# AolinFeng/PMP-VVC-TIP2023

Hardware: AMD Instinct MI355X
Metric: CTUs/sec (luma QT+MTT inference+post-proc) (higher is better)
Workload: dtype f16x3

## Files before the change

### pmp_vvc_tip2023_amd/csrc/conv_f16x3.hip

```cpp
#include <cstdio>
#include <type_traits>

#include "pmp_kernels.h"
#include "split3.h"

namespace pmp {

template <int KH, int KW, int NTHR = 256>
struct StagePlanH {
    unsigned off[GeoH<KH, KW, 16, NTHR>::NLD];
    unsigned valid;
};

template <int KH, int KW, int NTHR = 256>
__device__ __forceinline__ void h2_plan(StagePlanH<KH, KW, NTHR> &p, size_t plane_stride, int H, int W, int ty, int tx)
{
    typedef GeoH<KH, KW, 16, NTHR> G;
    constexpr int PY = KH / 2, PX = KW / 2;
    p.valid = 0;
#pragma unroll
    for (int k = 0; k < G::NLD; ++k) {
        const int i = min((int)threadIdx.x + k * NTHR, G::PIECES - 1);
        const int sp = i / G::PLANE, j = i - sp * G::PLANE, pix = j >> 1, half = j & 1;
        const int row = pix / G::TW, col = pix - row * G::TW;
        const int gy = ty * 16 + row - PY, gx = tx * 16 + col - PX;
        const bool in = gy >= 0 && gy < H && gx >= 0 && gx < W && (int)threadIdx.x + k * NTHR < G::PIECES;
        if (in) p.valid |= 1u << k;
        const int cy = min(max(gy, 0), H - 1), cx = min(max(gx, 0), W - 1);
        p.off[k] = (unsigned)(sp * plane_stride + ((size_t)cy * W + cx) * 16 + half * 8);
    }
}

template <int KH, int KW, int NTHR = 256>
__device__ __forceinline__ void h2_stage_load(const StagePlanH<KH, KW, NTHR> &p, const unsigned short *__restrict__ grp,
                                              u32x4 (&r)[GeoH<KH, KW, 16, NTHR>::NLD], int k0 = 0, int k1 = 1 << 20)
{
#pragma unroll
    for (int k = 0; k < GeoH<KH, KW, 16, NTHR>::NLD; ++k) {
        if (k < k0 || k >= k1) continue;
        r[k] = *reinterpret_cast<const u32x4 *>(grp + p.off[k]);
    }
}

template <int KH, int KW, int NTHR = 256>
__device__ __forceinline__ void h2_stage_store(const StagePlanH<KH, KW, NTHR> &p, u32x4 *lds, const u32x4 (&r)[GeoH<KH, KW, 16, NTHR>::NLD],
                                               int k0 = 0, int k1 = 1 << 20)
{
    typedef GeoH<KH, KW, 16, NTHR> G;
#pragma unroll
    for (int k = 0; k < G::NLD; ++k) {
        if (k < k0 || k >= k1) continue;
        const int i = min((int)threadIdx.x + k * NTHR, G::PIECES);
        const u32x4 z = {0u, 0u, 0u, 0u};
        lds[i] = ((p.valid >> k) & 1u) ? r[k] : z;
    }
}

template <int KH, int KW, int NT, bool LEAN = false>
__device__ __forceinline__ void h2_accumulate(const unsigned short *__restrict__ x, size_t plane_stride,
                                              const unsigned short *__restrict__ wpk, int C, int H, int W, int n, int ty,
                                              int tx, u32x4 *lds, f32x4 (&acc)[WaveTile<NT>::RW][WaveTile<NT>::CW])
{
    constexpr int NTHR = 256;
    typedef GeoH<KH, KW, 16, NTHR> G;
    typedef WaveTile<NT> WT;
    constexpr int RW = WT::RW, CW = WT::CW;
    const int lane = threadIdx.x & 63, wave = threadIdx.x >> 6, xl = lane & 15, g = lane >> 4;
    const int rh = wave % WT::RSPLIT, ch = wave / WT::RSPLIT;
    const int CB = C >> 4;
    const size_t grp_sz = (size_t)H * W * 16;
    const unsigned short *grp0 = x + (size_t)n * CB * grp_sz;
    constexpr bool W0DB = NT == 4;
    constexpr bool W2 = W0DB && G::TAPS == 9 && !LEAN;
    u32x4 r[G::NLD];
    StagePlanH<KH, KW, NTHR> plan;
    const bool paired = (CB & 1) == 0 && (G::TAPS & 1);
    const f16x8 *wl = reinterpret_cast<const f16x8 *>(wpk) + lane + ch * CW * 64;
    const int last = paired ? (CB / 2) * G::TAPS - 1 : CB * G::NKS - 1;
    f16x8 w0[CW], w1[CW];
    f16x8 w0n[CW];
    f16x8 w1n[CW], w0nn[CW];
    h2_plan<KH, KW, NTHR>(plan, plane_stride, H, W, ty, tx);
#pragma unroll
    for (int nt = 0; nt < CW; ++nt) {
        if (W0DB) w0n[nt] = wl[(0 * NT + nt) * 64]; else w0[nt] = wl[(0 * NT + nt) * 64];
        w1[nt] = wl[(1 * NT + nt) * 64];
        if (W2) {
            const f16x8 *w2 = wl + (size_t)min(1, last) * (2 * NT * 64);
            w0nn[nt] = w2[(0 * NT + nt) * 64]; w1n[nt] = w2[(1 * NT + nt) * 64];
        }
    }
    __syncthreads();
    h2_stage_load<KH, KW, NTHR>(plan, grp0, r);
    h2_stage_store<KH, KW, NTHR>(plan, lds, r);
    __syncthreads();
    const int pb = ((rh * RW * G::TW + xl) * 2 + (g & 1)) * 16;
    int stream = 0;
    int tapsel = g >> 1;
    constexpr int O_LAST = (((G::TAPS - 1) / KW) * G::TW + (G::TAPS - 1) % KW) * 32;
    f16x8 x0[RW], x1[RW];

    auto group = [&](auto mode_tag, auto tail_tag, int cb) {
        constexpr int MODE = decltype(mode_tag)::value;
        constexpr int TAIL = decltype(tail_tag)::value;
        constexpr bool LAST = TAIL == 2;
        constexpr int NK = MODE == 0 ? G::NKS : (MODE == 1 ? (G::TAPS - 1) / 2 : (G::TAPS - 1) / 2 + 1);
        constexpr int PER = (G::NLD + (NK > 0 ? NK : 1) - 1) / (NK > 0 ? NK : 1);
        constexpr int LAG = G::TAPS > 9 ? 3 : 2;
        constexpr bool FETCH = TAIL < 2;
        u32x4 (&rl)[G::NLD] = r;
        u32x4 (&rs)[G::NLD] = r;
        constexpr bool more = !LAST;
        const unsigned short *nxt_grp = grp0 + (size_t)min(cb + 1, CB - 1) * grp_sz;
        const int bcur = cb & 1, bprev = (cb + 1) & 1;
        const char *buf = reinterpret_cast<const char *>(lds + bcur * G::BUF);
        auto xaddr = [&](int ks) -> const char * {
            const int j = MODE == 2 ? ks - 1 : ks;
            int tA = 2 * j, tB = 2 * j + 1;
            if (MODE == 0 && tB >= G::TAPS) tB = tA;
            const int oA = ((tA / KW) * G::TW + tA % KW) * 32, oB = ((tB / KW) * G::TW + tB % KW) * 32;
            return buf + (tapsel ? oB : oA) + pb;
        };
        if constexpr (LEAN) {
            constexpr int RS = 2, SUB = RW / RS;
            const char *part = reinterpret_cast<const char *>(lds + bprev * G::BUF);
            if (NK == 0 && FETCH) h2_stage_load<KH, KW, NTHR>(plan, nxt_grp, rl);
#pragma unroll
            for (int ks = 0; ks < NK; ++ks) {
                asm volatile("" : "+v"(tapsel));
                const char *px = (MODE == 2 && ks == 0) ? (g < 2 ? part : buf) + O_LAST + pb : xaddr(ks);
                ++stream;
                const f16x8 *wf = wl + (size_t)min(stream, last) * (2 * NT * 64);
                f16x8 xa[RS], xb[RS];
                auto rd_a = [&](int h) __attribute__((always_inline)) {
#pragma unroll
                    for (int m = 0; m < RS; ++m) xa[m] = *reinterpret_cast<const f16x8 *>(px + (h * RS + m) * G::TW * 32);
                };
                auto rd_b = [&](int h) __attribute__((always_inline)) {
#pragma unroll
                    for (int m = 0; m < RS; ++m) xb[m] = *reinterpret_cast<const f16x8 *>(px + G::PLANE * 16 + (h * RS + m) * G::TW * 32);
                };
#pragma unroll
                for (int h = 0; h < SUB; ++h) {
                    rd_a(h); rd_b(h);
                    __builtin_amdgcn_sched_barrier(0);
#pragma unroll
                    for (int m = 0; m < RS; ++m)
#pragma unroll
                        for (int nt = 0; nt < CW; ++nt)
                            acc[h * RS + m][nt] = __builtin_amdgcn_mfma_f32_16x16x32_f16(w1[nt], xa[m], acc[h * RS + m][nt], 0, 0, 0);
                    __builtin_amdgcn_sched_barrier(0);
                    if (h == 0) {
#pragma unroll
                        for (int nt = 0; nt < CW; ++nt) w0[nt] = w0n[nt];
#pragma unroll
                        for (int nt = 0; nt < CW; ++nt) { w1n[nt] = wf[(1 * NT + nt) * 64]; w0n[nt] = wf[(0 * NT + nt) * 64]; }
                        if (FETCH) h2_stage_load<KH, KW, NTHR>(plan, nxt_grp, rl, ks * PER, (ks + 1) * PER);
                        if (more && ks >= LAG)
                            h2_stage_store<KH, KW, NTHR>(plan, lds + ((cb + 1) & 1) * G::BUF, rs, (ks - LAG) * PER, (ks - LAG + 1) * PER);
                    } else if (h == SUB - 1) {
#pragma unroll
                        for (int nt = 0; nt < CW; ++nt) w1[nt] = w1n[nt];
                    }
                    __builtin_amdgcn_sched_barrier(0);
#pragma unroll
                    for (int m = 0; m < RS; ++m)
#pragma unroll
                        for (int nt = 0; nt < CW; ++nt)
                            acc[h * RS + m][nt] = __builtin_amdgcn_mfma_f32_16x16x32_f16(w0[nt], xa[m], acc[h * RS + m][nt], 0, 0, 0);
                    __builtin_amdgcn_sched_barrier(0);
#pragma unroll
                    for (int m = 0; m < RS; ++m)
#pragma unroll
                        for (int nt = 0; nt < CW; ++nt)
                            acc[h * RS + m][nt] = __builtin_amdgcn_mfma_f32_16x16x32_f16(w0[nt], xb[m], acc[h * RS + m][nt], 0, 0, 0);
                    __builtin_amdgcn_sched_barrier(0);
                }
                if (MODE == 2 && ks == 0) h2_lds_barrier();
            }
        } else {
            if (NK == 0) {
                if (FETCH) h2_stage_load<KH, KW, NTHR>(plan, nxt_grp, rl);
            } else if (MODE == 2) {
                if (g >= 2) {
                    const char *pl = buf + O_LAST + pb;
#pragma unroll
                    for (int m = 0; m < RW; ++m) {
                        x0[m] = *reinterpret_cast<const f16x8 *>(pl + m * G::TW * 32);
                        x1[m] = *reinterpret_cast<const f16x8 *>(pl + G::PLANE * 16 + m * G::TW * 32);
                    }
                }
            } else {
                const char *p0x = xaddr(0);
#pragma unroll
                for (int m = 0; m < RW; ++m) x0[m] = *reinterpret_cast<const f16x8 *>(p0x + m * G::TW * 32);
            }
#pragma unroll
            for (int ks = 0; ks < NK; ++ks) {
                asm volatile("" : "+v"(tapsel));
                const char *px = (MODE == 2 && ks == 0) ? buf : xaddr(ks);
                ++stream;
                if (!(MODE == 2 && ks == 0)) {
#pragma unroll
                    for (int m = 0; m < RW; ++m) x1[m] = *reinterpret_cast<const f16x8 *>(px + G::PLANE * 16 + m * G::TW * 32);
                }
                const f16x8 *wf = wl + (size_t)min(stream, last) * (2 * NT * 64);
                __builtin_amdgcn_sched_barrier(0);
#pragma unroll
                for (int m = 0; m < RW; ++m)
#pragma unroll
                    for (int nt = 0; nt < CW; ++nt) acc[m][nt] = __builtin_amdgcn_mfma_f32_16x16x32_f16(w1[nt], x0[m], acc[m][nt], 0, 0, 0);
                __builtin_amdgcn_sched_barrier(0);
                if (W2) {
                    const f16x8 *wf2 = wl + (size_t)min(stream + 1, last) * (2 * NT * 64);
#pragma unroll
                    for (int nt = 0; nt < CW; ++nt) { w1[nt] = w1n[nt]; w0[nt] = w0n[nt]; w0n[nt] = w0nn[nt]; }
#pragma unroll
                    for (int nt = 0; nt < CW; ++nt) w1n[nt] = wf2[(1 * NT + nt) * 64];
#pragma unroll
                    for (int nt = 0; nt < CW; ++nt) w0nn[nt] = wf2[(0 * NT + nt) * 64];
                } else {
#pragma unroll
                    for (int nt = 0; nt < CW; ++nt) w1[nt] = wf[(1 * NT + nt) * 64];
                    if (W0DB) {
#pragma unroll
                        for (int nt = 0; nt < CW; ++nt) w0[nt] = w0n[nt];
#pragma unroll
                        for (int nt = 0; nt < CW; ++nt) w0n[nt] = wf[(0 * NT + nt) * 64];
                    }
                }
                if (FETCH) h2_stage_load<KH, KW, NTHR>(plan, nxt_grp, rl, ks * PER, (ks + 1) * PER);
                if (more && ks >= LAG)
                    h2_stage_store<KH, KW, NTHR>(plan, lds + ((cb + 1) & 1) * G::BUF, rs, (ks - LAG) * PER, (ks - LAG + 1) * PER);
                __builtin_amdgcn_sched_barrier(0);
#pragma unroll
                for (int m = 0; m < RW; ++m)
#pragma unroll
                    for (int nt = 0; nt < CW; ++nt) acc[m][nt] = __builtin_amdgcn_mfma_f32_16x16x32_f16(w0[nt], x0[m], acc[m][nt], 0, 0, 0);
                __builtin_amdgcn_sched_barrier(0);
                if (ks + 1 < NK) {
                    const char *pn = xaddr(ks + 1);
#pragma unroll
                    for (int m = 0; m < RW; ++m) x0[m] = *reinterpret_cast<const f16x8 *>(pn + m * G::TW * 32);
                }
                __builtin_amdgcn_sched_barrier(0);
#pragma unroll
                for (int m = 0; m < RW; ++m)
#pragma unroll
                    for (int nt = 0; nt < CW; ++nt) acc[m][nt] = __builtin_amdgcn_mfma_f32_16x16x32_f16(w0[nt], x1[m], acc[m][nt], 0, 0, 0);
                __builtin_amdgcn_sched_barrier(0);
                if (!W0DB) {
#pragma unroll
                    for (int nt = 0; nt < CW; ++nt) w0[nt] = wf[(0 * NT + nt) * 64];
                }
                __builtin_amdgcn_sched_barrier(0);
            }
            if (MODE == 1 && g < 2) {
                const char *pl = buf + O_LAST + pb;
#pragma unroll
                for (int m = 0; m < RW; ++m) {
                    x0[m] = *reinterpret_cast<const f16x8 *>(pl + m * G::TW * 32);
                    x1[m] = *reinterpret_cast<const f16x8 *>(pl + G::PLANE * 16 + m * G::TW * 32);
                }
            }
        }
        if (more) h2_stage_store<KH, KW, NTHR>(plan, lds + ((cb + 1) & 1) * G::BUF, rs, NK > LAG ? (NK - LAG) * PER : 0);
        __syncthreads();
    };

    typedef std::integral_constant<int, 0> M0;
    typedef std::integral_constant<int, 1> M1;
    typedef std::integral_constant<int, 2> M2;
    typedef std::integral_constant<int, 0> T0;
    typedef std::integral_constant<int, 1> T1;
    typedef std::integral_constant<int, 2> T2;
    if (paired) {
        for (int cb = 0; cb + 2 < CB; cb += 2) {
            group(M1{}, T0{}, cb);
            group(M2{}, T0{}, cb + 1);
        }
        group(M1{}, T1{}, CB - 2);
        group(M2{}, T2{}, CB - 1);
    } else {
        for (int cb = 0; cb + 1 < CB; ++cb) group(M0{}, T0{}, cb);
        group(M0{}, T2{}, CB - 1);
    }
}

template <int NT>
__device__ __forceinline__ void h2_epilogue(const ConvX6Args &a, f32x4 (&acc)[WaveTile<NT>::RW][WaveTile<NT>::CW], int n, int ty, int tx);

template <int NT>
__device__ __forceinline__ void h2_shortcut32(const ConvX6Args &a, int n, int ty, int tx, u32x4 *lds,
                                              f32x4 (&acc)[WaveTile<NT>::RW][WaveTile<NT>::CW])
{
    typedef WaveTile<NT> WT;
    constexpr int RW = WT::RW, CW = WT::CW;
    const int tid = threadIdx.x, lane = tid & 63, wave = tid >> 6, xl = lane & 15, g = lane >> 4;
    const int rh = wave % WT::RSPLIT, ch = wave / WT::RSPLIT;
    const int W = a.W;
    const size_t grp_sz = (size_t)a.H * W * 16;
    const unsigned short *base = a.x_sc + (size_t)n * 2 * grp_sz + ((size_t)(ty * 16) * W + tx * 16) * 16;
    __syncthreads();
    u32x4 r[8];
#pragma unroll
    for (int k = 0; k < 8; ++k) {
        const int i = tid + k * 256, grp = i >> 10, plane = (i >> 9) & 1, j = i & 511, px = j >> 1, half = j & 1;
        r[k] = *reinterpret_cast<const u32x4 *>(base + plane * a.sc_stride + grp * grp_sz + ((size_t)(px >> 4) * W + (px & 15)) * 16 + half * 8);
    }
    const f16x8 *wl = reinterpret_cast<const f16x8 *>(a.w_sc) + lane + ch * CW * 64;
    f16x8 w0[CW], w1[CW];
#pragma unroll
    for (int nt = 0; nt < CW; ++nt) { w0[nt] = wl[(0 * NT + nt) * 64]; w1[nt] = wl[(1 * NT + nt) * 64]; }
#pragma unroll
    for (int k = 0; k < 8; ++k) lds[tid + k * 256] = r[k];
    __syncthreads();
    const char *px = reinterpret_cast<const char *>(lds) + (g >> 1) * 16384 + ((rh * RW * 16 + xl) * 2 + (g & 1)) * 16;
#pragma unroll
    for (int h = 0; h < RW / 2; ++h) {
        f16x8 xa[2], xb[2];
#pragma unroll
        for (int m = 0; m < 2; ++m) {
            xa[m] = *reinterpret_cast<const f16x8 *>(px + (h * 2 + m) * 16 * 32);
            xb[m] = *reinterpret_cast<const f16x8 *>(px + 8192 + (h * 2 + m) * 16 * 32);
        }
#pragma unroll
        for (int m = 0; m < 2; ++m)
#pragma unroll
            for (int nt = 0; nt < CW; ++nt) acc[h * 2 + m][nt] = __builtin_amdgcn_mfma_f32_16x16x32_f16(w1[nt], xa[m], acc[h * 2 + m][nt], 0, 0, 0);
#pragma unroll
        for (int m = 0; m < 2; ++m)
#pragma unroll
            for (int nt = 0; nt < CW; ++nt) acc[h * 2 + m][nt] = __builtin_amdgcn_mfma_f32_16x16x32_f16(w0[nt], xa[m], acc[h * 2 + m][nt], 0, 0, 0);
#pragma unroll
        for (int m = 0; m < 2; ++m)
#pragma unroll
            for (int nt = 0; nt < CW; ++nt) acc[h * 2 + m][nt] = __builtin_amdgcn_mfma_f32_16x16x32_f16(w0[nt], xb[m], acc[h * 2 + m][nt], 0, 0, 0);
    }
}

template <int KH, int KW, int NT, int SC, bool LEAN = false>
__global__ __launch_bounds__(256, NT == 4 && !LEAN ? 2 : 3) void conv_h2_kernel(ConvX6Args a)
{
    typedef GeoH<KH, KW> G;
    __shared__ u32x4 lds[2 * G::BUF];
    const int tiles_x = a.W >> 4, tiles = tiles_x * (a.H >> 4);
    int bid = blockIdx.x;
    if ((gridDim.x & 7) == 0) bid = (bid & 7) * (gridDim.x >> 3) + (bid >> 3);
    const int n = bid / tiles, t = bid - n * tiles, ty = t / tiles_x, tx = t - ty * tiles_x;
    typedef WaveTile<NT> WT;
    constexpr int RW = WT::RW, CW = WT::CW;

    f32x4 acc[RW][CW];
#pragma unroll
    for (int m = 0; m < RW; ++m)
#pragma unroll
        for (int nt = 0; nt < CW; ++nt) acc[m][nt] = (f32x4){0.f, 0.f, 0.f, 0.f};

    h2_accumulate<KH, KW, NT, LEAN>(a.x, a.x_stride, a.w, a.Cin, a.H, a.W, n, ty, tx, lds, acc);
    if (SC == 2) h2_shortcut32<NT>(a, n, ty, tx, lds, acc);
    else if (SC) h2_accumulate<1, 1, NT, LEAN>(a.x_sc, a.sc_stride, a.w_sc, a.Csc, a.H, a.W, n, ty, tx, lds, acc);
    h2_epilogue<NT>(a, acc, n, ty, tx);
}

template <int NT>
__device__ __forceinline__ void h2_epilogue(const ConvX6Args &a, f32x4 (&acc)[WaveTile<NT>::RW][WaveTile<NT>::CW], int n, int ty, int tx)
{
    typedef WaveTile<NT> WT;
    constexpr int RW = WT::RW, CW = WT::CW;
    int tid = threadIdx.x;
    asm volatile("" : "+v"(tid));
    const int lane = tid & 63, wave = tid >> 6, xl = lane & 15, g = lane >> 4;
    const int rh = wave % WT::RSPLIT, ch = wave / WT::RSPLIT;
    const int H = a.H, W = a.W;
    const size_t grp = (size_t)H * W * 16;

    const float inv_scale = a.out_scale;
    const unsigned off0 = (unsigned)(((size_t)n * NT + ch * CW) * grp + ((size_t)(ty * 16 + rh * RW) * W + tx * 16 + xl) * 16 + g * 4);
    const unsigned row_el = (unsigned)W * 16;
    const unsigned off0w = off0 - (unsigned)(g * 4) + (unsigned)(8 * (g >> 1)) + (unsigned)(g & 1) * row_el;
    u32x4 ra[RW / 2][CW], rbv[RW / 2][CW];
    auto res_load = [&](int nt, int slot) __attribute__((always_inline)) {
#pragma unroll
        for (int m = 0; m < RW; m += 2) {
            const unsigned off = off0w + (unsigned)m * row_el + (unsigned)nt * (unsigned)grp;
            ra[m >> 1][slot] = __builtin_nontemporal_load(reinterpret_cast<const u32x4 *>(a.res + off));
            rbv[m >> 1][slot] = __builtin_nontemporal_load(reinterpret_cast<const u32x4 *>(a.res + off + a.res_stride));
        }
    };
    auto res_add = [&](int nt, int slot) __attribute__((always_inline)) {
#pragma unroll
        for (int m = 0; m < RW; m += 2) {
            u32x4 p = ra[m >> 1][slot], q = rbv[m >> 1][slot];
            rows16_swap(p);
            rows16_swap(q);
            acc[m][nt] = acc[m][nt] * inv_scale + h2_sum4_lo(p, q);
            acc[m + 1][nt] = acc[m + 1][nt] * inv_scale + h2_sum4_hi(p, q);
        }
    };
    if (a.res) {
#pragma unroll
        for (int nt = 0; nt < CW; ++nt) res_load(nt, nt);
#pragma unroll
        for (int nt = 0; nt < CW; ++nt) res_add(nt, nt);
    } else {
#pragma unroll
        for (int nt = 0; nt < CW; ++nt)
#pragma unroll
            for (int m = 0; m < RW; ++m) acc[m][nt] = acc[m][nt] * inv_scale;
    }
    float amax = 0.f;
#pragma unroll
    for (int nt = 0; nt < CW; ++nt) {
#pragma unroll
        for (int m = 0; m < RW; ++m) {
            const unsigned off = off0 + (unsigned)m * row_el + (unsigned)nt * (unsigned)grp;
            f32x4 v = acc[m][nt];
            if (a.relu) { v.x = fmaxf(v.x, 0.f); v.y = fmaxf(v.y, 0.f); v.z = fmaxf(v.z, 0.f); v.w = fmaxf(v.w, 0.f); }
            if (a.gate) v *= load_split2_4(a.gate + off, a.gate_stride);
            amax = sat_amax4(amax, v);
            acc[m][nt] = v;
        }
        if (!a.pool) {
            if (a.out_f32) {
#pragma unroll
                for (int m = 0; m < RW; ++m)
                    *reinterpret_cast<f32x4 *>(a.out_f32 + off0 + (unsigned)m * row_el + (unsigned)nt * (unsigned)grp) = acc[m][nt];
            } else {
#pragma unroll
                for (int m = 0; m < RW; m += 2) {
                    const unsigned off = off0w + (unsigned)m * row_el + (unsigned)nt * (unsigned)grp;
                    u32x4 p, q;
                    split2_rows(acc[m][nt], acc[m + 1][nt], p, q);
                    rows16_swap(p);
                    rows16_swap(q);
                    __builtin_nontemporal_store(p, reinterpret_cast<u32x4 *>(a.out + off));
                    __builtin_nontemporal_store(q, reinterpret_cast<u32x4 *>(a.out + off + a.out_stride));
                }
            }
        } else {
            const int Ho = H >> 1, Wo = W >> 1;
#pragma unroll
            for (int m = 0; m < RW; m += 2) {
                f32x4 v = acc[m][nt], u = acc[m + 1][nt];
                v.x = fmaxf(v.x, u.x); v.y = fmaxf(v.y, u.y); v.z = fmaxf(v.z, u.z); v.w = fmaxf(v.w, u.w);
                f32x4 o;
                o.x = __shfl_xor(v.x, 1); o.y = __shfl_xor(v.y, 1); o.z = __shfl_xor(v.z, 1); o.w = __shfl_xor(v.w, 1);
                v.x = fmaxf(v.x, o.x); v.y = fmaxf(v.y, o.y); v.z = fmaxf(v.z, o.z); v.w = fmaxf(v.w, o.w);
                if ((xl & 1) == 0) {
                    const int yo = ty * 8 + rh * (RW / 2) + (m >> 1), xo = tx * 8 + (xl >> 1);
                    const size_t off = (((size_t)n * NT + ch * CW + nt) * Ho + yo) * Wo * 16 + (size_t)xo * 16 + g * 4;
                    if (a.out_f32) *reinterpret_cast<f32x4 *>(a.out_f32 + off) = v;
                    else store_split2_4(a.out + off, a.out_stride, v);
                }
            }
        }
    }
    if (!a.out_f32) sat_report(a.sat, amax);
}

#define PMP_H2_LAUNCH(NT)                                                                                       \
    if (a.x_sc) hipLaunchKernelGGL((conv_h2_kernel<KH, KW, NT, 1>), dim3(grid), dim3(256), 0, s, a);           \
    else hipLaunchKernelGGL((conv_h2_kernel<KH, KW, NT, 0>), dim3(grid), dim3(256), 0, s, a)

template <int KH, int KW>
static hipError_t launch_h2(hipStream_t s, const ConvX6Args &a)
{
    const int grid = a.N * (a.H >> 4) * (a.W >> 4);
    switch (a.Cout >> 4) {
    case 1: PMP_H2_LAUNCH(1); break;
    case 2: PMP_H2_LAUNCH(2); break;
    case 4:
        if constexpr (KH > 1) {
            if (a.x_sc && a.Csc == 32) {
                hipLaunchKernelGGL((conv_h2_kernel<KH, KW, 4, 2>), dim3(grid), dim3(256), 0, s, a);
                break;
            }
            if (!a.x_sc) {
                hipLaunchKernelGGL((conv_h2_kernel<KH, KW, 4, 0, true>), dim3(grid), dim3(256), 0, s, a);
                break;
            }
        }
        PMP_H2_LAUNCH(4);
        break;
    default: return hipErrorInvalidValue;
    }
    return hipGetLastError();
}
#undef PMP_H2_LAUNCH

hipError_t launch_conv_h2(hipStream_t s, const ConvX6Args &a_in)
{
    const ConvX6Args &a = a_in;

    if ((a.H & 15) || (a.W & 15) || (a.Cin & 15) || (a.Cout & 15) || (a.x_sc && (a.Csc & 15)) || a.N <= 0)
        return hipErrorInvalidValue;
    if (a.pool && a.gate) return hipErrorInvalidValue;
    if (!(a.out_scale > 0.f)) return hipErrorInvalidValue;
    if (a.KH == 3 && a.KW == 3) return launch_h2<3, 3>(s, a);
    if (a.KH == 5 && a.KW == 5) return launch_h2<5, 5>(s, a);
    if (a.KH == 1 && a.KW == 1) return launch_h2<1, 1>(s, a);
    return hipErrorInvalidValue;
}

__global__ __launch_bounds__(256) void f32_to_split2_kernel(const float *__restrict__ x, unsigned short *__restrict__ out,
                                                            size_t n4, size_t plane_stride, unsigned *sat)
{
    float amax = 0.f;
    for (size_t i = (size_t)blockIdx.x * 256 + threadIdx.x; i < n4; i += (size_t)gridDim.x * 256) {
        const f32x4 v = *reinterpret_cast<const f32x4 *>(x + i * 4);
        amax = sat_amax4(amax, v);
        store_split2_4(out + i * 4, plane_stride, v);
    }
    sat_report(sat, amax);
}

__global__ __launch_bounds__(256) void split2_to_f32_kernel(const unsigned short *__restrict__ x, float *__restrict__ out,
                                                            size_t n4, size_t plane_stride)
{
    for (size_t i = (size_t)blockIdx.x * 256 + threadIdx.x; i < n4; i += (size_t)gridDim.x * 256)
        *reinterpret_cast<f32x4 *>(out + i * 4) = load_split2_4(x + i * 4, plane_stride);
}

hipError_t launch_f32_to_split2(hipStream_t s, const float *x, unsigned short *out, size_t n, size_t plane_stride, unsigned *sat)
{
    const size_t n4 = n / 4;
    const unsigned grid = (unsigned)((n4 + 255) / 256 > 16384 ? 16384 : (n4 + 255) / 256);
    if (n4) hipLaunchKernelGGL(f32_to_split2_kernel, dim3(grid), dim3(256), 0, s, x, out, n4, plane_stride, sat);
    return hipGetLastError();
}

hipError_t launch_split2_to_f32(hipStream_t s, const unsigned short *x, float *out, size_t n, size_t plane_stride)
{
    const size_t n4 = n / 4;
    const unsigned grid = (unsigned)((n4 + 255) / 256 > 16384 ? 16384 : (n4 + 255) / 256);
    if (n4) hipLaunchKernelGGL(split2_to_f32_kernel, dim3(grid), dim3(256), 0, s, x, out, n4, plane_stride);
    return hipGetLastError();
}

}
```

Baseline: 15520.

## Stage conv input tiles with global_load_lds DMA and explicit vmcnt waits

Adds a DMA path for the Cout=64 LEAN convolution kernels that copies input halo tiles straight from global memory into LDS with global_load_lds_dwordx4, so they no longer pass through registers and a separate LDS store. Out-of-bounds pieces point at a zeroed global line. Weight loads become inline-asm global loads with hand-counted vmcnt waits, interleaved with the DMA slices across the k-steps. This is meant to cut VGPR pressure and LDS-store instructions in the pipelined loop. It adds fragile manual waitcnt accounting and changes the shortcut-32 kernel from non-LEAN to LEAN+DMA, which also raises its occupancy bound from 2 to 3.

```diff
diff --git a/pmp_vvc_tip2023_amd/csrc/conv_f16x3.hip b/pmp_vvc_tip2023_amd/csrc/conv_f16x3.hip
--- a/pmp_vvc_tip2023_amd/csrc/conv_f16x3.hip
+++ b/pmp_vvc_tip2023_amd/csrc/conv_f16x3.hip
@@ -56,13 +56,114 @@
     }
 }
 
-template <int KH, int KW, int NT, bool LEAN = false>
+__device__ u32x4 h2_zero_line[1];
+
+template <int KH, int KW>
+struct DmaPlanH {
+    typedef GeoH<KH, KW, 16, 256, true> G;
+    static constexpr int NQW = (G::NQ + 3) / 4;
+    static constexpr bool KEEP = KH * KW <= 9;
+    unsigned off[KEEP ? NQW : 1];
+    unsigned valid;
+    size_t plane_stride;
+    int H, W, ty, tx;
+};
+
+template <int KH, int KW>
+__device__ __forceinline__ bool h2_dma_piece(int k, int lane, int wave, size_t plane_stride, int H, int W, int ty, int tx, unsigned &off)
+{
+    typedef typename DmaPlanH<KH, KW>::G G;
+    constexpr int PY = KH / 2, PX = KW / 2;
+    const int i = min(wave + 4 * k, G::NQ - 1) * 64 + lane, ic = min(i, G::PIECES - 1);
+    const int sp = ic / G::PLANE, j = ic - sp * G::PLANE, pix = j >> 1, half = j & 1;
+    const int row = pix / G::TW, col = pix - row * G::TW;
+    const int gy = ty * 16 + row - PY, gx = tx * 16 + col - PX;
+    off = (unsigned)(sp * plane_stride + ((size_t)max(gy, 0) * W + max(gx, 0)) * 16 + half * 8);
+    return i < G::PIECES && gy >= 0 && gy < H && gx >= 0 && gx < W;
+}
+
+template <int KH, int KW>
+__device__ __forceinline__ void h2_dma_plan(DmaPlanH<KH, KW> &p, size_t plane_stride, int H, int W, int ty, int tx)
+{
+    const int lane = threadIdx.x & 63, wave = threadIdx.x >> 6;
+    p.valid = 0;
+    p.plane_stride = plane_stride; p.H = H; p.W = W; p.ty = ty; p.tx = tx;
+    if constexpr (DmaPlanH<KH, KW>::KEEP) {
+#pragma unroll
+        for (int k = 0; k < DmaPlanH<KH, KW>::NQW; ++k)
+            if (h2_dma_piece<KH, KW>(k, lane, wave, plane_stride, H, W, ty, tx, p.off[k])) p.valid |= 1u << k;
+    }
+}
+
+__device__ __forceinline__ void h2_dma16(const void *src, unsigned lds_byte)
+{
+    unsigned keep;
+    asm volatile("s_mov_b32 %0, m0\n\ts_mov_b32 m0, %2\n\ts_nop 0\n\tglobal_load_lds_dwordx4 %1, off\n\ts_mov_b32 m0, %0"
+                 : "=&s"(keep) : "v"(src), "s"(lds_byte) : "memory");
+}
+
+template <int KH, int KW>
+__device__ __forceinline__ void h2_dma_issue(const DmaPlanH<KH, KW> &p, const unsigned short *grp, unsigned lds_buf, int k0, int k1)
+{
+    typedef typename DmaPlanH<KH, KW>::G G;
+    const int wave = __builtin_amdgcn_readfirstlane(threadIdx.x >> 6);
+#pragma unroll
+    for (int k = 0; k < DmaPlanH<KH, KW>::NQW; ++k) {
+        if (k < k0 || k >= k1) continue;
+        bool in;
+        unsigned off;
+        if constexpr (DmaPlanH<KH, KW>::KEEP) {
+            in = (p.valid >> k) & 1u;
+            off = p.off[k];
+        } else {
+            int lane = threadIdx.x & 63;
+            asm volatile("" : "+v"(lane));
+            in = h2_dma_piece<KH, KW>(k, lane, wave, p.plane_stride, p.H, p.W, p.ty, p.tx, off);
+        }
+        const void *src = in ? (const void *)(grp + off) : (const void *)h2_zero_line;
+        h2_dma16(src, lds_buf + (unsigned)(min(wave + 4 * k, G::NQ - 1) * 1024));
+    }
+}
+
+__device__ __forceinline__ void h2_wload(f16x8 &dst, const f16x8 *src)
+{
+    asm volatile("global_load_dwordx4 %0, %1, off" : "=v"(dst) : "v"(src) : "memory");
+}
+
+template <int N>
+__device__ __forceinline__ void h2_wwait_c(f16x8 (&w)[2])
+{
+    asm volatile("s_waitcnt vmcnt(%c2)" : "+v"(w[0]), "+v"(w[1]) : "i"(N) : "memory");
+}
+
+__device__ __forceinline__ void h2_wwait(int n, f16x8 (&w)[2])
+{
+    switch (n) {
+    case 0: h2_wwait_c<0>(w); break;
+    case 1: h2_wwait_c<1>(w); break;
+    case 2: h2_wwait_c<2>(w); break;
+    case 3: h2_wwait_c<3>(w); break;
+    case 4: h2_wwait_c<4>(w); break;
+    case 5: h2_wwait_c<5>(w); break;
+    case 6: h2_wwait_c<6>(w); break;
+    default: h2_wwait_c<0>(w); break;
+    }
+}
+
+template <int N>
+__device__ __forceinline__ void h2_wait_barrier()
+{
+    asm volatile("s_waitcnt vmcnt(%c0) lgkmcnt(0)\n\ts_barrier" :: "i"(N) : "memory");
+}
+
+template <int KH, int KW, int NT, bool LEAN = false, bool DMA = false>
 __device__ __forceinline__ void h2_accumulate(const unsigned short *__restrict__ x, size_t plane_stride,
                                               const unsigned short *__restrict__ wpk, int C, int H, int W, int n, int ty,
                                               int tx, u32x4 *lds, f32x4 (&acc)[WaveTile<NT>::RW][WaveTile<NT>::CW])
 {
     constexpr int NTHR = 256;
-    typedef GeoH<KH, KW, 16, NTHR> G;
+    static_assert(!DMA || (LEAN && NT == 4), "the DMA form is a LEAN form at Cout = 64");
+    typedef GeoH<KH, KW, 16, NTHR, DMA> G;
     typedef WaveTile<NT> WT;
     constexpr int RW = WT::RW, CW = WT::CW;
     const int lane = threadIdx.x & 63, wave = threadIdx.x >> 6, xl = lane & 15, g = lane >> 4;
@@ -80,20 +181,32 @@
     f16x8 w0[CW], w1[CW];
     f16x8 w0n[CW];
     f16x8 w1n[CW], w0nn[CW];
-    h2_plan<KH, KW, NTHR>(plan, plane_stride, H, W, ty, tx);
-#pragma unroll
-    for (int nt = 0; nt < CW; ++nt) {
-        if (W0DB) w0n[nt] = wl[(0 * NT + nt) * 64]; else w0[nt] = wl[(0 * NT + nt) * 64];
-        w1[nt] = wl[(1 * NT + nt) * 64];
-        if (W2) {
-            const f16x8 *w2 = wl + (size_t)min(1, last) * (2 * NT * 64);
-            w0nn[nt] = w2[(0 * NT + nt) * 64]; w1n[nt] = w2[(1 * NT + nt) * 64];
-        }
-    }
-    __syncthreads();
-    h2_stage_load<KH, KW, NTHR>(plan, grp0, r);
-    h2_stage_store<KH, KW, NTHR>(plan, lds, r);
-    __syncthreads();
+    DmaPlanH<KH, KW> dplan;
+    const unsigned lds_byte = (unsigned)(size_t)(__attribute__((address_space(3))) char *)lds;
+    if constexpr (DMA) {
+        h2_dma_plan<KH, KW>(dplan, plane_stride, H, W, ty, tx);
+#pragma unroll
+        for (int nt = 0; nt < CW; ++nt) { h2_wload(w0n[nt], wl + (0 * NT + nt) * 64); h2_wload(w1[nt], wl + (1 * NT + nt) * 64); }
+        __syncthreads();
+        h2_dma_issue<KH, KW>(dplan, grp0, lds_byte, 0, DmaPlanH<KH, KW>::NQW);
+        asm volatile("s_waitcnt vmcnt(0)" : "+v"(w0n[0]), "+v"(w0n[1]), "+v"(w1[0]), "+v"(w1[1]) :: "memory");
+        h2_wait_barrier<0>();
+    } else {
+        h2_plan<KH, KW, NTHR>(plan, plane_stride, H, W, ty, tx);
+#pragma unroll
+        for (int nt = 0; nt < CW; ++nt) {
+            if (W0DB) w0n[nt] = wl[(0 * NT + nt) * 64]; else w0[nt] = wl[(0 * NT + nt) * 64];
+            w1[nt] = wl[(1 * NT + nt) * 64];
+            if (W2) {
+                const f16x8 *w2 = wl + (size_t)min(1, last) * (2 * NT * 64);
+                w0nn[nt] = w2[(0 * NT + nt) * 64]; w1n[nt] = w2[(1 * NT + nt) * 64];
+            }
+        }
+        __syncthreads();
+        h2_stage_load<KH, KW, NTHR>(plan, grp0, r);
+        h2_stage_store<KH, KW, NTHR>(plan, lds, r);
+        __syncthreads();
+    }
     const int pb = ((rh * RW * G::TW + xl) * 2 + (g & 1)) * 16;
     int stream = 0;
     int tapsel = g >> 1;
@@ -108,6 +221,12 @@
         constexpr int PER = (G::NLD + (NK > 0 ? NK : 1) - 1) / (NK > 0 ? NK : 1);
         constexpr int LAG = G::TAPS > 9 ? 3 : 2;
         constexpr bool FETCH = TAIL < 2;
+        constexpr int NQW = DmaPlanH<KH, KW>::NQW;
+        constexpr int DS = MODE == 2 ? 1 : 0;
+        constexpr int DPER = (NQW + (NK > DS ? NK - DS : 1) - 1) / (NK > DS ? NK - DS : 1);
+        constexpr int KD = DS + (NQW + DPER - 1) / DPER - 1;
+        static_assert(!DMA || (NK > DS && KD < NK), "DMA slices must fit the group");
+        auto ndma = [](int ks) { return ks < DS ? 0 : max(0, min(NQW, (ks - DS + 1) * DPER) - (ks - DS) * DPER); };
         u32x4 (&rl)[G::NLD] = r;
         u32x4 (&rs)[G::NLD] = r;
         constexpr bool more = !LAST;
@@ -124,6 +243,7 @@
         if constexpr (LEAN) {
             constexpr int RS = 2, SUB = RW / RS;
             const char *part = reinterpret_cast<const char *>(lds + bprev * G::BUF);
+            const unsigned nxt_lds = lds_byte + (unsigned)(((cb + 1) & 1) * G::BUF * 16);
             if (NK == 0 && FETCH) h2_stage_load<KH, KW, NTHR>(plan, nxt_grp, rl);
 #pragma unroll
             for (int ks = 0; ks < NK; ++ks) {
@@ -150,7 +270,20 @@
                         for (int nt = 0; nt < CW; ++nt)
                             acc[h * RS + m][nt] = __builtin_amdgcn_mfma_f32_16x16x32_f16(w1[nt], xa[m], acc[h * RS + m][nt], 0, 0, 0);
                     __builtin_amdgcn_sched_barrier(0);
-                    if (h == 0) {
+                    if (h == 0 && DMA) {
+                        h2_wwait(ks == 0 || !FETCH ? 0 : ndma(ks - 1), w0n);
+#pragma unroll
+                        for (int nt = 0; nt < CW; ++nt) w0[nt] = w0n[nt];
+#pragma unroll
+                        for (int nt = 0; nt < CW; ++nt) h2_wload(w1n[nt], wf + (1 * NT + nt) * 64);
+#pragma unroll
+                        for (int nt = 0; nt < CW; ++nt) h2_wload(w0n[nt], wf + (0 * NT + nt) * 64);
+                        if (FETCH) h2_dma_issue<KH, KW>(dplan, nxt_grp, nxt_lds, (ks - DS) * DPER, ks < DS ? 0 : (ks - DS + 1) * DPER);
+                    } else if (h == SUB - 1 && DMA) {
+                        h2_wwait(CW + (FETCH ? ndma(ks) : 0), w1n);
+#pragma unroll
+                        for (int nt = 0; nt < CW; ++nt) w1[nt] = w1n[nt];
+                    } else if (h == 0) {
 #pragma unroll
                         for (int nt = 0; nt < CW; ++nt) w0[nt] = w0n[nt];
 #pragma unroll
@@ -264,8 +397,13 @@
                 }
             }
         }
-        if (more) h2_stage_store<KH, KW, NTHR>(plan, lds + ((cb + 1) & 1) * G::BUF, rs, NK > LAG ? (NK - LAG) * PER : 0);
-        __syncthreads();
+        if constexpr (DMA) {
+            if constexpr (FETCH) h2_wait_barrier<2 * CW * (NK - 1 - KD)>();
+            else h2_lds_barrier();
+        } else {
+            if (more) h2_stage_store<KH, KW, NTHR>(plan, lds + ((cb + 1) & 1) * G::BUF, rs, NK > LAG ? (NK - LAG) * PER : 0);
+            __syncthreads();
+        }
     };
 
     typedef std::integral_constant<int, 0> M0;
@@ -285,6 +423,7 @@
         for (int cb = 0; cb + 1 < CB; ++cb) group(M0{}, T0{}, cb);
         group(M0{}, T2{}, CB - 1);
     }
+    if constexpr (DMA) asm volatile("s_waitcnt vmcnt(0)" : "+v"(w0n[0]), "+v"(w0n[1]), "+v"(w1n[0]), "+v"(w1n[1]) :: "memory");
 }
 
 template <int NT>
@@ -339,10 +478,10 @@
     }
 }
 
-template <int KH, int KW, int NT, int SC, bool LEAN = false>
+template <int KH, int KW, int NT, int SC, bool LEAN = false, bool DMA = false>
 __global__ __launch_bounds__(256, NT == 4 && !LEAN ? 2 : 3) void conv_h2_kernel(ConvX6Args a)
 {
-    typedef GeoH<KH, KW> G;
+    typedef GeoH<KH, KW, 16, 256, DMA> G;
     __shared__ u32x4 lds[2 * G::BUF];
     const int tiles_x = a.W >> 4, tiles = tiles_x * (a.H >> 4);
     int bid = blockIdx.x;
@@ -357,7 +496,7 @@
 #pragma unroll
         for (int nt = 0; nt < CW; ++nt) acc[m][nt] = (f32x4){0.f, 0.f, 0.f, 0.f};
 
-    h2_accumulate<KH, KW, NT, LEAN>(a.x, a.x_stride, a.w, a.Cin, a.H, a.W, n, ty, tx, lds, acc);
+    h2_accumulate<KH, KW, NT, LEAN, DMA>(a.x, a.x_stride, a.w, a.Cin, a.H, a.W, n, ty, tx, lds, acc);
     if (SC == 2) h2_shortcut32<NT>(a, n, ty, tx, lds, acc);
     else if (SC) h2_accumulate<1, 1, NT, LEAN>(a.x_sc, a.sc_stride, a.w_sc, a.Csc, a.H, a.W, n, ty, tx, lds, acc);
     h2_epilogue<NT>(a, acc, n, ty, tx);
@@ -473,11 +612,11 @@
     case 4:
         if constexpr (KH > 1) {
             if (a.x_sc && a.Csc == 32) {
-                hipLaunchKernelGGL((conv_h2_kernel<KH, KW, 4, 2>), dim3(grid), dim3(256), 0, s, a);
+                hipLaunchKernelGGL((conv_h2_kernel<KH, KW, 4, 2, true, true>), dim3(grid), dim3(256), 0, s, a);
                 break;
             }
             if (!a.x_sc) {
-                hipLaunchKernelGGL((conv_h2_kernel<KH, KW, 4, 0, true>), dim3(grid), dim3(256), 0, s, a);
+                hipLaunchKernelGGL((conv_h2_kernel<KH, KW, 4, 0, true, true>), dim3(grid), dim3(256), 0, s, a);
                 break;
             }
         }
```

Result: no change. 15640 (median of 6 runs) (+0.7%).
